# Developer-Zer0/GIF-synthesis-with-Discrete-Diffusion

Measured on AMD Instinct MI355X. Metric: 16-frame 128x128 videos/sec, 100-step D3PM sample, higher is better.
Workload: dtype f32; 1 GPU; C3: D3PM 100-step p_sample, guidance 2, 16x16x16 token grid, K=4096, 19 layers, bs 16/GPU + VQ-VAE decode to 3x16x128x128; global_batch=16, parallelism=replicas x1 (batch-sharded, no collective), hipgraph=True, sampler_lanes=2, weights=reference init N(0, 0.02)

## Files before the change

### gif-synthesis-with-discrete-diffusion_amd/_lib.py

```python
import ctypes as C
import os

import torch

_HERE = os.path.dirname(os.path.abspath(__file__))
LIB_PATH = os.environ.get("GSDD_LIB_PATH") or os.path.join(_HERE, "libgsdd.so")
_lib = None

EXPORTS = [
    "gsdd_last_error", "gsdd_version", "gsdd_abi_sizeof", "gsdd_gemm", "gsdd_row_stats", "gsdd_ncdhw_to_rows", "gsdd_preprocess_clip",
    "gsdd_axial_attention", "gsdd_pool3d", "gsdd_nearest_code", "gsdd_nearest_code_workspace_bytes", "gsdd_bn_train_workspace_bytes", "gsdd_bn_train",
    "gsdd_codebook_ema", "gsdd_code_perplexity", "gsdd_mse", "gsdd_conv_wgrad", "gsdd_bn_relu_bwd_workspace_bytes", "gsdd_bn_relu_bwd",
    "gsdd_relu_mask", "gsdd_lincomb", "gsdd_axial_attention_bwd", "gsdd_d3pm_embed", "gsdd_adaln_table", "gsdd_small_linear",
    "gsdd_d3pm_attention", "gsdd_d3pm_attention_workspace_bytes", "gsdd_d3pm_layer", "gsdd_d3pm_layer_pack", "gsdd_d3pm_layer_pack_h2", "gsdd_rows_linear_pack_many", "gsdd_rows_linear", "gsdd_d3pm_logits", "gsdd_d3pm_cross_attention", "gsdd_d3pm_step", "gsdd_d3pm_q_sample", "gsdd_d3pm_train_loss", "gsdd_d3pm_train_loss_bwd", "gsdd_d3pm_train_loss_grad", "gsdd_gelu2", "gsdd_ln_fwd", "gsdd_ln_bwd", "gsdd_wgrad",
    "gsdd_batch_rowsum", "gsdd_colsum", "gsdd_d3pm_attention_train", "gsdd_d3pm_attention_bwd", "gsdd_d3pm_attention_bwd_workspace_bytes", "gsdd_d3pm_embed_bwd", "gsdd_small_linear_bwd",
    "gsdd_adaln_bwd", "gsdd_adam", "gsdd_adam_multi", "gsdd_adam_multi_dev", "gsdd_advance", "gsdd_advance_floor",
    "gsdd_d3pm_purity_step", "gsdd_d3pm_purity_select", "gsdd_advance_plan",
    "gsdd_philox_uniform", "gsdd_graph_begin", "gsdd_graph_end", "gsdd_graph_launch", "gsdd_graph_destroy",
    "gsdd_event_create", "gsdd_event_record", "gsdd_event_elapsed_ms", "gsdd_event_destroy",
]

_p = C.c_void_p
_i = C.c_int
_i64 = C.c_int64
# ... 32 lines not shown
    ]


class PuritySelectDesc(C.Structure):
    _fields_ = [
        ("tok_in", _p), ("tok_out", _p), ("cand", _p), ("score", _p), ("smax", _p),
        ("B", _i), ("L", _i), ("K", _i), ("prior_rule", _i), ("n_dev", _p), ("seed", C.c_uint64), ("stream_dev", _p),
        ("stream_add", _i64), ("row0", _i64), ("key_dbg", _p),
    ]


class TrainDesc(C.Structure):
    _fields_ = [
        ("logits", _p), ("x0", _p), ("xt", _p), ("t_dev", _p), ("pt", _p),
        ("B", _i), ("L", _i), ("K", _i), ("T", _i), ("sched", _p * 8), ("mask_weight", C.c_float * 2),
        ("aux_weight", C.c_float), ("adaptive_aux", _i),
        ("kl", _p), ("nll", _p), ("aux", _p), ("x0_recon", _p), ("xt1_recon", _p),
        ("Lt_history", _p), ("Lt_count", _p), ("loss", _p), ("per_sample", _p), ("probs", _p),
    ]


class LayerDesc(C.Structure):
    _fields_ = [
        ("y", _p), ("x", _p), ("M", _i64), ("L", _i), ("n_embd", _i), ("hidden", _i), ("cvec", _p),
        ("wproj", _p), ("bproj", _p), ("ln2_g", _p), ("ln2_b", _p), ("w1", _p), ("b1", _p), ("w2", _p), ("b2", _p),
        ("ada", _p), ("t2", _p), ("wqkv", _p), ("bqkv", _p), ("qkv", _p), ("w2_x3", _p), ("wqkv_x3", _p), ("kv_img_bytes", _i64), ("kv_img", _p),
        ("layer_h2", _p), ("wqkv_h2", _p), ("variant", _i), ("range_flag", _p),
    ]


GEMM_EXACT_F32 = 1
AXIAL_AUTO, AXIAL_VALU = 0, 1
ATTN_AUTO, ATTN_P22, ATTN_P11, ATTN_A8, ATTN_A12, ATTN_F32PV, ATTN_KC256 = range(7)
LAYER_AUTO, LAYER_X3P, LAYER_H2 = 0, 2, 3
ATTN_BWD_AUTO, ATTN_BWD_VALU, ATTN_BWD_SPLIT, ATTN_BWD_FQC64, ATTN_BWD_FQC128, ATTN_BWD_NW8, ATTN_BWD_DBG1, ATTN_BWD_DBG2 = range(8)


class GsddError(RuntimeError):
    pass


def lib():
    global _lib
    if _lib is None:
        if not os.path.exists(LIB_PATH):
            raise GsddError(f"{LIB_PATH} is missing: the HIP extension must be built (./build.sh); "
                            "there is no CPU fallback for this path")
        L = C.CDLL(LIB_PATH)
        L.gsdd_last_error.restype = C.c_char_p
        if not hasattr(L, "gsdd_abi_sizeof"):
            raise GsddError(f"{LIB_PATH} predates this binding (no gsdd_abi_sizeof): rebuild it with ./build.sh")
        L.gsdd_abi_sizeof.argtypes, L.gsdd_abi_sizeof.restype = [_i], _i64
        for which, (name, cls) in enumerate((("gsdd_gemm_desc", GemmDesc), ("gsdd_layer_desc", LayerDesc), ("gsdd_step_desc", StepDesc),
                                             ("gsdd_train_desc", TrainDesc), ("gsdd_purity_desc", PurityDesc),
                                             ("gsdd_purity_select_desc", PuritySelectDesc))):
            if L.gsdd_abi_sizeof(which) != C.sizeof(cls):
                raise GsddError(f"{LIB_PATH} was built from another revision of include/gsdd.h: sizeof({name}) is {L.gsdd_abi_sizeof(which)} "
                                f"there and {C.sizeof(cls)} in this binding -- rebuild it with ./build.sh")
        L.gsdd_gemm.argtypes = [C.POINTER(GemmDesc), _p]
        L.gsdd_row_stats.argtypes = [_p, _i64, _i, C.c_float, _p, _p]
        L.gsdd_ncdhw_to_rows.argtypes = [_p, _i, _i, _i, _i, _i, _i, _i, _p, _p]
        L.gsdd_preprocess_clip.argtypes = [_p] + [_i] * 10 + [_p, _p]
        L.gsdd_axial_attention.argtypes = [_p, _i, _i, _i, _i, _i, _i, _p, _i, _p]
        L.gsdd_pool3d.argtypes = [_p, _i, _i, _i, _i, _i, _i, C.POINTER(_i), C.POINTER(_i), C.POINTER(_i), _i, _i, _i, _i, _p, _i, _p]
        L.gsdd_nearest_code.argtypes = [_p, _i64, _i, _p, _i, _p, _p, _p, _i64, _p]
        L.gsdd_nearest_code_workspace_bytes.argtypes = [_i]
# ... 85 lines not shown
```

### gif-synthesis-with-discrete-diffusion_amd/csrc/common.hpp

```cpp
#pragma once
#include <hip/hip_runtime.h>
#include <stdint.h>
#include <stdio.h>
#include <string.h>
#include <atomic>
#include <string>

#include "../../include/gsdd.h"

namespace gsdd {

void set_error(const std::string& s);

#define GSDD_CHECK_ARG(cond, msg)                                                      \
    do {                                                                               \
        if (!(cond)) {                                                                 \
            ::gsdd::set_error(std::string(__func__) + ": " + (msg) + " [" #cond "]"); \
            return GSDD_E_ARG;                                                         \
        }                                                                              \
    } while (0)

#define GSDD_CHECK_HIP(expr)                                                                   \
    do {                                                                                       \
        hipError_t e_ = (expr);                                                                \
// ... 101 lines not shown
        const float r1 = (vs[d] - (float)a) * 2048.f;
        const _Float16 b2 = (_Float16)r1;
        const float r2 = (r1 - (float)b2) * 2048.f;
        col[d] = a; col[4 + d] = b2; col[8 + d] = (_Float16)r2;
    }
    col[12] = (_Float16)1.f;
    col[13] = col[14] = col[15] = (_Float16)0.f;
    const int64_t pair = row >> 5;
    const int kk = (int)(row & 31), th = kk >> 4, kt = kk & 15, g = kt >> 2, r = kt & 3;
    _Float16* dst = reinterpret_cast<_Float16*>(vp + (pair * 4 + g) * 16) + 4 * th + r;
#pragma unroll
    for (int j = 0; j < 16; ++j) dst[j * 8] = col[j];
}

__host__ __device__ __forceinline__ float4* kv_image_ksum(void* workspace, int64_t rows) {
    return reinterpret_cast<float4*>(reinterpret_cast<char*>(workspace) + rows * 64);
}
__host__ __device__ __forceinline__ float* kv_image_knorm(void* workspace, int64_t rows) {
    return reinterpret_cast<float*>(reinterpret_cast<char*>(workspace) + rows * 64 + ((rows + 31) / 32) * 16);
}
template <int CTRL>
__device__ __forceinline__ float dpp_max(float v) {
    return fmaxf(v, __int_as_float(__builtin_amdgcn_update_dpp(0, __float_as_int(v), CTRL, 0xf, 0xf, true)));
}
template <int CTRL>
__device__ __forceinline__ float dpp_min(float v) {
    return fminf(v, __int_as_float(__builtin_amdgcn_update_dpp(__float_as_int(v), __float_as_int(v), CTRL, 0xf, 0xf, false)));
}
__device__ __forceinline__ float row16_max(float v) {
    v = dpp_max<0xB1>(v);
    v = dpp_max<0x4E>(v);
    v = dpp_max<0x141>(v);
    return dpp_max<0x140>(v);
}
__device__ __forceinline__ float row16_min(float v) {
    v = dpp_min<0xB1>(v);
    v = dpp_min<0x4E>(v);
    v = dpp_min<0x141>(v);
    return dpp_min<0x140>(v);
}
template <int CTRL>
__device__ __forceinline__ float dpp_add(float v) {
    return v + __int_as_float(__builtin_amdgcn_update_dpp(0, __float_as_int(v), CTRL, 0xf, 0xf, true));
}
__device__ __forceinline__ float dpp_prev_row_lane15(float v) {
    return __int_as_float(__builtin_amdgcn_update_dpp(0, __float_as_int(v), 0x142, 0xa, 0xf, false));
}
__device__ __forceinline__ float half32_sum(float v) {
    v = dpp_add<0xB1>(v);
    v = dpp_add<0x4E>(v);
    v = dpp_add<0x141>(v);
    v = dpp_add<0x140>(v);
    return v + dpp_prev_row_lane15(v);
}
__device__ __forceinline__ float half32_norm_bound(float n2) {
    float v = row16_max(n2);
    v = fmaxf(v, dpp_prev_row_lane15(v));
    return sqrtf(v) * 1.000001f + 1e-30f;
}
__device__ __forceinline__ void kv_image_store_knorm(const float4 (&o)[8], int h, int li, int64_t grp, int64_t M, float* knorm,
                                                     float4* ksum) {
#pragma unroll
    for (int q = 0; q < 8; ++q) {
        const float n2 = (o[q].x * o[q].x + o[q].y * o[q].y) + (o[q].z * o[q].z + o[q].w * o[q].w);
        const float nb = half32_norm_bound(n2);
        const float4 sk = make_float4(half32_sum(o[q].x), half32_sum(o[q].y), half32_sum(o[q].z), half32_sum(o[q].w));
// ... 16 lines not shown
```

### gif-synthesis-with-discrete-diffusion_amd/csrc/d3pm_attention.hip

```cpp
#include <stdlib.h>

#include <type_traits>

#include "common.hpp"

namespace gsdd {

typedef float f32x4 __attribute__((ext_vector_type(4)));
typedef __bf16 bf16x8 __attribute__((ext_vector_type(8)));

constexpr int KC = 256;
constexpr float RESCALE_THR = 40.f;

struct AttnSmem {
    uint4 k[2][KC][2];
    float v[2][KC / 4][4][4];
    uint4 ones[16];
};

__device__ __forceinline__ bf16x8 as_frag(uint4 u) {
    union { uint4 u; bf16x8 v; } c;
    c.u = u;
    return c.v;
}
// ... 313 lines not shown
            float p[8];
#pragma unroll
            for (int r = 0; r < 4; ++r) { p[r] = __builtin_amdgcn_exp2f(s0[r]); p[4 + r] = __builtin_amdgcn_exp2f(s1[r]); }
            uint4 hi, lo;
            if (MODE == 1) {
                split_p8(p, hi, lo);
                acc[j] = __builtin_amdgcn_mfma_f32_16x16x32_f16(as_h8(hi), vb, acc[j], 0, 0, 0);
                acc[j] = __builtin_amdgcn_mfma_f32_16x16x32_f16(as_h8(lo), vb, acc[j], 0, 0, 0);
            } else {
                round_p8(p, hi);
                acc[j] = __builtin_amdgcn_mfma_f32_16x16x32_f16(as_h8(hi), vb, acc[j], 0, 0, 0);
                if (MODE == 2) {
                    if (!MASK || !((skipmask[j] >> u) & 1u)) {
                        if (!MEASURE || __any(any_gt_h8(hi, thr2[j]))) {
                            resid_p8(p, hi, lo);
                            acc[j] = __builtin_amdgcn_mfma_f32_16x16x32_f16(as_h8(lo), vb, acc[j], 0, 0, 0);
                        } else {
                            ++skipped;
                        }
                    }
                }
            }
        }
    }
    return skipped;
}


template <int KC4, int PM = 1>
__global__ __launch_bounds__(256) void d3pm_attention_v4_kernel(const float* __restrict__ q, const uint4* __restrict__ kp,
                                                                const uint4* __restrict__ vp, const float* __restrict__ knorm,
                                                                const float4* __restrict__ ksum, int B, int L, int H,
                                                                float* __restrict__ out,
                                                                float* __restrict__ lse, unsigned long long* __restrict__ redo) {
    __shared__ AttnSmem4<KC4> sm;
    const int tid = threadIdx.x, lane = tid & 63, wave = tid >> 6;
    const int nqb = (L + 255) / 256;
    const unsigned nwg = gridDim.x;
    unsigned wg = blockIdx.x;
    {
        const unsigned q8 = nwg / 8, r8 = nwg % 8, xcd = wg % 8, idx = wg / 8;
        wg = (xcd < r8 ? xcd * (q8 + 1) : r8 * (q8 + 1) + (xcd - r8) * q8) + idx;
    }
    const int qblk = wg % nqb;
    const int h = (wg / nqb) % H, b = wg / (nqb * H);
    const int64_t M = (int64_t)B * L;
    const int64_t base = ((int64_t)h * M + (int64_t)b * L) * 4;
    const float* qh = q + base;
    const uint4* kph = kp + ((int64_t)h * M + (int64_t)b * L) * 2;
    const uint4* vph = vp + (((int64_t)h * M + (int64_t)b * L) >> 5) * 64;
    const float* knh = knorm + (((int64_t)h * M + (int64_t)b * L) >> 5);
    const float4* ksh = ksum + (((int64_t)h * M + (int64_t)b * L) >> 5);
    const int li = lane & 15, lg = lane >> 4;
    const int q0 = qblk * 256 + wave * 64;

    float knm = 0.f;
    float4 ks = make_float4(0.f, 0.f, 0.f, 0.f);
    if (PM >= 2) {
        for (int i = lane; i < (L >> 5); i += 64) {
            knm = fmaxf(knm, knh[i]);
            const float4 t = ksh[i];
            ks.x += t.x; ks.y += t.y; ks.z += t.z; ks.w += t.w;
        }
    }

    if (tid < 16) sm.ones[tid] = (tid == 0 || tid == 1) ? make_uint4(0x3F803F80u, 0x00003F80u, 0u, 0u) : make_uint4(0u, 0u, 0u, 0u);

    const float qscale = 0.5f * 1.4426950408889634f;
    uint4 qfrag[4];
    float rqn[4];
    float4 qsv[4];
#pragma unroll
    for (int j = 0; j < 4; ++j) {
        int qi = q0 + 16 * j + li;
        qi = qi < L ? qi : L - 1;
        const float4 qv = *reinterpret_cast<const float4*>(qh + (int64_t)qi * 4);
        const float qs[4] = {qv.x * qscale, qv.y * qscale, qv.z * qscale, qv.w * qscale};
        uint32_t q1[4], q2[4], q3[4];
#pragma unroll
        for (int d = 0; d < 4; ++d) split3(qs[d], q1[d], q2[d], q3[d]);
        const uint4 f0 = pack8(q1, q1), f1 = pack8(q2, q2), f2 = pack8(q1, q3);
        qfrag[j] = lg == 0 ? f0 : (lg == 1 ? f1 : (lg == 2 ? f2 : make_uint4(0u, 0u, 0u, 0u)));
        rqn[j] = 1.0f / (sqrtf((qs[0] * qs[0] + qs[1] * qs[1]) + (qs[2] * qs[2] + qs[3] * qs[3])) * 1.0001f + 1e-30f);
        qsv[j] = make_float4(qs[0], qs[1], qs[2], qs[3]);
    }

    const int nchunks = (L + KC4 - 1) / KC4;
    uint4 rk0, rk1, rk2, rv0, rv1, rv2;
    float rkn = 0.f, kn_cur = 0.f;
    auto load_chunk = [&](int c) {
        const int last = 2 * min(KC4, L - c * KC4) - 1;
        const uint4* ksrc = kph + (int64_t)c * KC4 * 2;
        const uint4* vsrc = vph + (int64_t)c * (KC4 / 32) * 64;
        rk0 = ksrc[min(tid, last)]; rk1 = ksrc[min(tid + 256, last)]; rk2 = ksrc[min(tid + 512, last)];
        rv0 = vsrc[min(tid, last)]; rv1 = vsrc[min(tid + 256, last)]; rv2 = vsrc[min(tid + 512, last)];
        if (PM >= 2) rkn = knh[min(c * (KC4 / 32) + min(lane, KC4 / 32 - 1), (L >> 5) - 1)];
    };
    auto store_chunk = [&](int buf, int) {
        uint4* kd = &sm.k[buf][0][0];
        uint4* vd = &sm.v[buf][0][0][0];
        kd[tid] = rk0; kd[tid + 256] = rk1; kd[tid + 512] = rk2;
        vd[tid] = rv0; vd[tid + 256] = rv1; vd[tid + 512] = rv2;
        kn_cur = rkn;
    };

    f32x4 acc[4], sav[4];
    float mq[4];
#pragma unroll
    for (int j = 0; j < 4; ++j) {
        mq[j] = 0.f;
        acc[j][0] = 0.f; acc[j][1] = 0.f; acc[j][2] = 0.f; acc[j][3] = 0.f;
    }
    const f32x4 zero = {0.f, 0.f, 0.f, 0.f};

    load_chunk(0);
    store_chunk(0, 0);
    __syncthreads();
    const int slot = ((lg >> 1) ^ (li >> 3)) & 1;
    const uint4* kbase0 = (lg == 3) ? &sm.ones[(li >= 4 && li < 12) ? 0 : 1] : &sm.k[0][li][slot];
    const int kstep = (lg == 3) ? 0 : 32;
    const int kbuf = (lg == 3) ? 0 : KC4 * 2;
    {
        const int nt0 = min(4, L >> 4);
#pragma unroll
        for (int j = 0; j < 4; ++j) {
            float m0 = -INFINITY;
            for (int t = 0; t < nt0; ++t) {
                const f32x4 s = __builtin_amdgcn_mfma_f32_16x16x32_bf16(as_frag(kbase0[t * kstep]), as_frag(qfrag[j]), zero, 0, 0, 0);
                m0 = fmaxf(m0, fmaxf(fmaxf(s[0], s[1]), fmaxf(s[2], s[3])));
            }
            m0 = fmaxf(m0, __shfl_xor(m0, 16));
            m0 = fmaxf(m0, __shfl_xor(m0, 32));
            mq[j] = ceilf(m0) - 3.f;
            if (lg == 3) qfrag[j] = negm_frag(mq[j]);
        }
    }

    bool prescan = false;
    bool adapt = PM >= 2;
    int probe = 1, backoff = 4;
    float jb[4] = {-INFINITY, -INFINITY, -INFINITY, -INFINITY};
    float kbj[4] = {0.f, 0.f, 0.f, 0.f};
    int kb_next = 1, kb_gap = 1;
    if (PM >= 2) {
        knm = wave_max(knm) * 1.0001f;
        const float budget = log2f((float)L) - (float)PM - 0.02f;
        ks.x = wave_sum(ks.x); ks.y = wave_sum(ks.y); ks.z = wave_sum(ks.z); ks.w = wave_sum(ks.w);
        const float invL = 1.0f / (float)L;
#pragma unroll
        for (int j = 0; j < 4; ++j) {
            const float dx = qsv[j].x * ks.x, dy = qsv[j].y * ks.y, dz = qsv[j].z * ks.z, dw = qsv[j].w * ks.w;
            const float mean = ((dx + dy) + (dz + dw)) * invL, mag = ((fabsf(dx) + fabsf(dy)) + (fabsf(dz) + fabsf(dw))) * invL;
            jb[j] = log2f((float)L) + mean - 1e-5f * mag - 0.02f;
            kbj[j] = row16_min(fmaxf(fmaxf(budget * rqn[j] - knm, (jb[j] - (float)PM) * rqn[j]), 0.f));
        }
    }
    for (int c = 0; c < nchunks; ++c) {
        const int buf = c & 1;
        if (c + 1 < nchunks) load_chunk(c + 1);
        const int npairs = min(KC4, L - c * KC4) >> 5;
        const uint4* kb = kbase0 + buf * kbuf;
#pragma unroll
        for (int j = 0; j < 4; ++j) sav[j] = acc[j];
        bool moved = false;
        for (int attempt = prescan ? -1 : 0; attempt < 16; ++attempt) {
          if (attempt >= 0) {
            uint32_t thr2[4] = {0u, 0u, 0u, 0u};
            uint32_t skipmask[4] = {0u, 0u, 0u, 0u};
            const uint32_t allmask = (1u << npairs) - 1u;
            if (PM >= 2) {
#pragma unroll
                for (int j = 0; j < 4; ++j) skipmask[j] = (uint32_t)__ballot(kn_cur < kbj[j]);
                const bool stale_clears = (skipmask[0] & skipmask[1] & skipmask[2] & skipmask[3] & allmask) == allmask;
                const bool refresh = !stale_clears && c >= kb_next;
                if (refresh) { kb_next = c + kb_gap; kb_gap *= 2; }
                if (refresh || (adapt && !stale_clears)) {
#pragma unroll
                    for (int j = 0; j < 4; ++j) {
                        const int src = ((li >> 2) << 4) + 12;
                        const float r0 = __shfl(sav[j][0], src), r1 = __shfl(sav[j][1], src), r2 = __shfl(sav[j][2], src),
                                    r3 = __shfl(sav[j][3], src);
                        const int rr = li & 3;
                        const float rs = rr == 0 ? r0 : (rr == 1 ? r1 : (rr == 2 ? r2 : r3));
                        if (refresh) {
                            float kbq = (__builtin_amdgcn_logf(rs) - (float)PM + mq[j] - 0.02f) * rqn[j];
                            kbq = fmaxf(kbq, 0.f);
                            kbj[j] = fmaxf(kbj[j], row16_min(kbq));

                            skipmask[j] = (uint32_t)__ballot(kn_cur < kbj[j]);
                        }
                        if (adapt && !stale_clears) {
                            const float rlb = fmaxf(rs, __builtin_amdgcn_exp2f(jb[j] - mq[j]));
// ... 2 lines not shown
                            thr2[j] = hb | (hb << 16);
                        }
                    }
                }
            }
            const uint32_t clr_all = skipmask[0] & skipmask[1] & skipmask[2] & skipmask[3] & allmask;
            int ncleared = 0;
#pragma unroll
            for (int j = 0; j < 4; ++j) ncleared += __builtin_popcount(skipmask[j] & allmask);
            int skipped = 0;
            const bool cleared = PM >= 2 && clr_all == allmask;
            if (PM == 0 || cleared) attn_tiles<KC4, 0>(sm, buf, npairs, kb, kstep, lg, li, qfrag, acc, thr2, skipmask);
            else if (PM == 1 || (!adapt && 2 * ncleared < 4 * npairs))
                attn_tiles<KC4, 1>(sm, buf, npairs, kb, kstep, lg, li, qfrag, acc, thr2, skipmask);
            else if (!adapt) skipped = ncleared + attn_tiles<KC4, 2, true, false>(sm, buf, npairs, kb, kstep, lg, li, qfrag, acc, thr2, skipmask);
            else if (ncleared == 0) skipped = attn_tiles<KC4, 2, false, true>(sm, buf, npairs, kb, kstep, lg, li, qfrag, acc, thr2, skipmask);
            else skipped = ncleared + attn_tiles<KC4, 2, true, true>(sm, buf, npairs, kb, kstep, lg, li, qfrag, acc, thr2, skipmask);
            float chk = 0.f;
#pragma unroll
            for (int j = 0; j < 4; ++j) chk += (acc[j][0] + acc[j][1]) + (acc[j][2] + acc[j][3]);
            const bool bad = !(fabsf(chk) < 3.0e38f);
            if (!__any(bad)) {
                if (PM >= 2 && !cleared) {
                    if (adapt) {
                        if (10 * skipped < 7 * 4 * npairs) { adapt = false; probe = backoff; backoff *= 2; }
                    } else if (--probe <= 0) {
                        adapt = true;
                    }
                }
                break;
            }
            moved = true;
            if (lane == 0 && redo != nullptr) atomicAdd(redo, 1ull);
          }
            const float trigger = attempt < 0 ? 12.f : 15.f;
            float cmax[4] = {-INFINITY, -INFINITY, -INFINITY, -INFINITY};
            for (int t = 0; t < 2 * npairs; ++t) {
                const bf16x8 kf = as_frag(kb[t * kstep]);
#pragma unroll
                for (int j = 0; j < 4; ++j) {
                    const f32x4 sx = __builtin_amdgcn_mfma_f32_16x16x32_bf16(kf, as_frag(qfrag[j]), zero, 0, 0, 0);
                    cmax[j] = fmaxf(cmax[j], fmaxf(fmaxf(sx[0], sx[1]), fmaxf(sx[2], sx[3])));
                }
            }
#pragma unroll
            for (int j = 0; j < 4; ++j) {
                float cm = fmaxf(cmax[j], __shfl_xor(cmax[j], 16));
                cm = fmaxf(cm, __shfl_xor(cm, 32));
                const float delta = cm >= trigger ? ceilf(cm) - 3.f : 0.f;
                if (attempt < 0 && __any(delta != 0.f)) moved = true;
                mq[j] += delta;
                if (lg == 3) qfrag[j] = negm_frag(mq[j]);
#pragma unroll
                for (int r = 0; r < 4; ++r) {
                    const float dr = __shfl(delta, (lane & 48) + 4 * lg + r);
                    acc[j][r] = sav[j][r] * __builtin_amdgcn_exp2f(-dr);
                }
                sav[j] = acc[j];
            }
        }
        prescan = moved;
        if (c + 1 < nchunks) store_chunk(buf ^ 1, c + 1);
        __syncthreads();
    }

#pragma unroll
    for (int j = 0; j < 4; ++j) {
#pragma unroll
        for (int r = 0; r < 4; ++r) {
            const float a = acc[j][r];
            const int rowbase = lane & 48;
            const float a1 = __shfl(a, rowbase + (li & 3) + 4);
            const float a2 = __shfl(a, rowbase + (li & 3) + 8);
            const float l = __shfl(a, rowbase + 12);
            const float mrow = __shfl(mq[j], rowbase + 4 * lg + r);
            const int qi = q0 + 16 * j + 4 * lg + r;
            if (li < 4 && qi < L) {
                const float o = (a + a1 * 0.00048828125f + a2 * 2.384185791015625e-07f) / l;
                out[((int64_t)b * L + qi) * (H * 4) + h * 4 + li] = o;
                if (lse != nullptr && li == 0) lse[(int64_t)h * M + (int64_t)b * L + qi] = mrow + log2f(l);
            }
        }
    }
}

__global__ void d3pm_cross_attention_kernel(const float* q, const float* kc, const float* vc, int B, int L, int Te, int H,
                                            float* out) {
    const int64_t M = (int64_t)B * L;
    const int64_t i = (int64_t)blockIdx.x * blockDim.x + threadIdx.x;
    if (i >= M * H) return;
    const int h = (int)(i / M);
    const int64_t m = i % M;
    const int b = (int)(m / L);
    const float4 qv = *reinterpret_cast<const float4*>(q + ((int64_t)h * M + m) * 4);
    float mx = -INFINITY;
    for (int e = 0; e < Te; ++e) {
        const float4 kv = *reinterpret_cast<const float4*>(kc + ((int64_t)b * Te + e) * (H * 4) + h * 4);
        const float s = (qv.x * kv.x + qv.y * kv.y + qv.z * kv.z + qv.w * kv.w) * 0.5f;
        mx = fmaxf(mx, s);
    }
    float l = 0.f, a0 = 0.f, a1 = 0.f, a2 = 0.f, a3 = 0.f;
    for (int e = 0; e < Te; ++e) {
        const float4 kv = *reinterpret_cast<const float4*>(kc + ((int64_t)b * Te + e) * (H * 4) + h * 4);
        const float4 vv = *reinterpret_cast<const float4*>(vc + ((int64_t)b * Te + e) * (H * 4) + h * 4);
        const float s = (qv.x * kv.x + qv.y * kv.y + qv.z * kv.z + qv.w * kv.w) * 0.5f;
        const float p = expf(s - mx);
        l += p;
        a0 += p * vv.x; a1 += p * vv.y; a2 += p * vv.z; a3 += p * vv.w;
    }
    const float inv = 1.0f / l;
    *reinterpret_cast<float4*>(out + m * (H * 4) + h * 4) = make_float4(a0 * inv, a1 * inv, a2 * inv, a3 * inv);
}

}

using namespace gsdd;

static int attn_p_mode(int mode, int L) {
    switch (mode) {
        case GSDD_ATTN_P22: return 1;
        case GSDD_ATTN_P11: return 0;
        case GSDD_ATTN_A8: return 8;
        case GSDD_ATTN_A12: return 12;
        default: return L >= 2048 ? 8 : 1;
    }
}

extern "C" int64_t gsdd_d3pm_attention_workspace_bytes(int B, int L, int H) {
    const int64_t rows = (int64_t)B * L * H;
    return rows * 64 + ((rows + 31) / 32) * 20;
}

int gsdd_attention_valu(const float* q, const float* k, const float* v, int B, int L, int H, float* out, float* lse,
                        void* stream);

extern "C" int gsdd_d3pm_attention(const float* q, const float* k, const float* v, int B, int L, int H, float* out,
                                   void* workspace, int64_t workspace_bytes, uint64_t* redo_events, int mode, void* stream) {
    GSDD_CHECK_ARG(q && out && ((k == nullptr) == (v == nullptr)), "null pointer");
    GSDD_CHECK_ARG(mode >= GSDD_ATTN_AUTO && mode <= GSDD_ATTN_KC256, "mode: one of GSDD_ATTN_*");
    GSDD_CHECK_ARG(B > 0 && H > 0 && L > 0, "bad sizes");
    GSDD_CHECK_ARG((int64_t)B * H * ((L + 255) / 256) < (1ll << 31), "grid too large");
    const bool premade = k == nullptr;
    const bool force_v3 = mode == GSDD_ATTN_F32PV;
    GSDD_CHECK_ARG(!premade || (L % 32 == 0 && workspace != nullptr && !force_v3), "k = v = NULL needs the matrix-pipe kernel's images in the workspace");
    if (L % 16 != 0) return gsdd_attention_valu(q, k, v, B, L, H, out, nullptr, stream);
    const dim3 grid((unsigned)(B * H * ((L + 255) / 256)));
    hipStream_t st = (hipStream_t)stream;
    if (L % 32 == 0 && !force_v3 && workspace != nullptr) {
        GSDD_CHECK_ARG(workspace_bytes >= gsdd_d3pm_attention_workspace_bytes(B, L, H), "workspace too small");
        const int64_t rows = (int64_t)B * L * H;
        uint4* kp = reinterpret_cast<uint4*>(workspace);
        uint4* vp = kp + rows * 2;
        float* kn = kv_image_knorm(workspace, rows);
        float4* ksm = kv_image_ksum(workspace, rows);
        unsigned long long* redo = reinterpret_cast<unsigned long long*>(redo_events);
        if (!premade) {
            hipLaunchKernelGGL(d3pm_attn_prep_kernel, dim3((unsigned)((rows + 255) / 256)), dim3(256), 0, st, k, v, rows, kp, vp, kn, ksm);
            GSDD_CHECK_LAUNCH();
        }
        const bool kc256 = mode == GSDD_ATTN_KC256;
        const int pmode = attn_p_mode(mode, L);
        float* nolse = nullptr;
        if (kc256) hipLaunchKernelGGL(d3pm_attention_v4_kernel<256>, grid, dim3(256), 0, st, q, kp, vp, kn, ksm, B, L, H, out, nolse, redo);
        else if (pmode == 0) hipLaunchKernelGGL((d3pm_attention_v4_kernel<384, 0>), grid, dim3(256), 0, st, q, kp, vp, kn, ksm, B, L, H, out, nolse, redo);
        else if (pmode == 8) hipLaunchKernelGGL((d3pm_attention_v4_kernel<384, 8>), grid, dim3(256), 0, st, q, kp, vp, kn, ksm, B, L, H, out, nolse, redo);
        else if (pmode == 12) hipLaunchKernelGGL((d3pm_attention_v4_kernel<384, 12>), grid, dim3(256), 0, st, q, kp, vp, kn, ksm, B, L, H, out, nolse, redo);
        else hipLaunchKernelGGL(d3pm_attention_v4_kernel<384>, grid, dim3(256), 0, st, q, kp, vp, kn, ksm, B, L, H, out, nolse, redo);
    } else {
        hipLaunchKernelGGL(d3pm_attention_kernel, grid, dim3(256), 0, st, q, k, v, B, L, H, out);
    }
    GSDD_CHECK_LAUNCH();
    return GSDD_OK;
}

int gsdd_attention_v4_with_lse(const float* q, const float* k, const float* v, int B, int L, int H, float* out, float* lse,
                               void* workspace, int64_t workspace_bytes, int mode, void* stream, int* done) {
    *done = 0;
    GSDD_CHECK_ARG(mode == GSDD_ATTN_AUTO || mode == GSDD_ATTN_P22 || mode == GSDD_ATTN_A8,
                   "training forward: mode is GSDD_ATTN_AUTO, GSDD_ATTN_P22 or GSDD_ATTN_A8");
    if (L % 32 != 0 || workspace == nullptr) return GSDD_OK;
    GSDD_CHECK_ARG(workspace_bytes >= gsdd_d3pm_attention_workspace_bytes(B, L, H), "workspace too small");
    GSDD_CHECK_ARG((int64_t)B * H * ((L + 255) / 256) < (1ll << 31), "grid too large");
    hipStream_t st = (hipStream_t)stream;
    const int64_t rows = (int64_t)B * L * H;
    uint4* kp = reinterpret_cast<uint4*>(workspace);
    uint4* vp = kp + rows * 2;
    float* kn = kv_image_knorm(workspace, rows);
    float4* ksm = kv_image_ksum(workspace, rows);
    unsigned long long* noredo = nullptr;
    hipLaunchKernelGGL(d3pm_attn_prep_kernel, dim3((unsigned)((rows + 255) / 256)), dim3(256), 0, st, k, v, rows, kp, vp, kn, ksm);
    GSDD_CHECK_LAUNCH();
    if (mode == GSDD_ATTN_A8 || (mode == GSDD_ATTN_AUTO && L >= 2048))
        hipLaunchKernelGGL((d3pm_attention_v4_kernel<384, 8>), dim3((unsigned)(B * H * ((L + 255) / 256))), dim3(256), 0, st, q, kp, vp, kn, ksm,
                           B, L, H, out, lse, noredo);
    else
        hipLaunchKernelGGL(d3pm_attention_v4_kernel<384>, dim3((unsigned)(B * H * ((L + 255) / 256))), dim3(256), 0, st, q, kp, vp, kn, ksm,
                           B, L, H, out, lse, noredo);
    GSDD_CHECK_LAUNCH();
    *done = 1;
    return GSDD_OK;
}

extern "C" int gsdd_d3pm_cross_attention(const float* q, const float* kc, const float* vc, int B, int L, int Te, int H,
                                         float* out, void* stream) {
    GSDD_CHECK_ARG(q && kc && vc && out, "null pointer");
    GSDD_CHECK_ARG(B > 0 && L > 0 && Te > 0 && H > 0, "bad sizes");
    const int64_t n = (int64_t)B * L * H;
    hipLaunchKernelGGL(d3pm_cross_attention_kernel, dim3((unsigned)((n + 255) / 256)), dim3(256), 0, (hipStream_t)stream,
                       q, kc, vc, B, L, Te, H, out);
    GSDD_CHECK_LAUNCH();
    return GSDD_OK;
}
```

### gif-synthesis-with-discrete-diffusion_amd/ops.py

```python
import ctypes as C
import os

import torch

from . import _lib as abi
from ._lib import GemmDesc, GsddError, LayerDesc, PurityDesc, PuritySelectDesc, StepDesc, TrainDesc, check, lib, ptr, stream_ptr

ACT_NONE, ACT_RELU, ACT_GELU2 = 0, 1, 2


_ATTN_MODES = {"auto": abi.ATTN_AUTO, "22": abi.ATTN_P22, "11": abi.ATTN_P11, "a8": abi.ATTN_A8, "a12": abi.ATTN_A12,
               "f32pv": abi.ATTN_F32PV, "kc256": abi.ATTN_KC256}
_LAYER_VARIANTS = {"auto": abi.LAYER_AUTO, "h2": abi.LAYER_H2, "x3p": abi.LAYER_X3P}
_ATTN_BWD_VARIANTS = {"auto": abi.ATTN_BWD_AUTO, "valu": abi.ATTN_BWD_VALU, "split": abi.ATTN_BWD_SPLIT, "fqc64": abi.ATTN_BWD_FQC64,
                      "fqc128": abi.ATTN_BWD_FQC128, "nw8": abi.ATTN_BWD_NW8, "dbg1": abi.ATTN_BWD_DBG1, "dbg2": abi.ATTN_BWD_DBG2}


def _pick(table, value, what):
    if isinstance(value, int):
        return value
    try:
        return table[str(value).lower()]
    except KeyError:
        raise GsddError(f"{what}: {value!r} is not one of {sorted(table)}") from None


def attn_mode(mode=None):
    if mode is not None:
        return _pick(_ATTN_MODES, mode, "attention mode")
    if os.environ.get("GSDD_ATTN_V3"):
        return abi.ATTN_F32PV
    if os.environ.get("GSDD_ATTN_KC") == "256":
        return abi.ATTN_KC256
    return _pick(_ATTN_MODES, os.environ.get("GSDD_ATTN_P", "auto"), "GSDD_ATTN_P")


def attn_train_mode(mode=None):
    v = mode if mode is not None else os.environ.get("GSDD_ATTN_TRAIN_P", "auto")
    m = _pick(_ATTN_MODES, v, "GSDD_ATTN_TRAIN_P")
    if m not in (abi.ATTN_AUTO, abi.ATTN_P22, abi.ATTN_A8):
        raise GsddError(f"GSDD_ATTN_TRAIN_P: {v!r} is not one of '22', 'a8'")
    return m


def attn_bwd_variant(variant=None):
    return _pick(_ATTN_BWD_VARIANTS, variant if variant is not None else os.environ.get("GSDD_ATTN_BWD", "auto"), "GSDD_ATTN_BWD")


def layer_variant(variant=None):
    return _pick(_LAYER_VARIANTS, variant if variant is not None else os.environ.get("GSDD_LAYER", "auto"), "GSDD_LAYER")


def gemm_flags(exact_f32=None):
    if exact_f32 is None:
        exact_f32 = bool(os.environ.get("GSDD_GEMM_F32"))
    return abi.GEMM_EXACT_F32 if exact_f32 else 0


def axial_variant(valu=None):
    if valu is None:
        valu = bool(os.environ.get("GSDD_AXIAL_VALU"))
    return abi.AXIAL_VALU if valu else abi.AXIAL_AUTO


def taps_tensor(taps, device):
    return torch.tensor(taps, dtype=torch.int32, device=device).contiguous()


def gemm(inp, w, out, *, in_dims, out_grid, stride=(1, 1, 1), taps=None, ntaps=1, cin=None, in_pitch=None,
         gather=None, pro=None, ln=None, epi_scale=None, epi_shift=None, bvec=None, rows_per_batch=0, act=ACT_NONE,
         residual=None, out_dims=None, out_step=(1, 1, 1), out_off=(0, 0, 0), out_pitch=None, out_mode=0, cout=None,
         exact_f32=None, stream=None, _desc_only=False):
    d = GemmDesc()
    N, Di, Hi, Wi = in_dims
    d.in_ = ptr(inp)
# ... 118 lines not shown
    return out[0]


def d3pm_embed(tok, emb, pos, x, rep=1, stream=None):
    B, L = tok.shape
    check(lib().gsdd_d3pm_embed(ptr(tok), B, L, emb.shape[1], ptr(emb), emb.shape[0], ptr(pos), rep, ptr(x),
                                stream_ptr(stream)))
    return x


def adaln_table(emb_w, lin_w, lin_b, out=None, stream=None):
    T, D = emb_w.shape
    if out is None:
        out = torch.empty((T, 2 * D), dtype=torch.float32, device=emb_w.device)
    check(lib().gsdd_adaln_table(ptr(emb_w), T, D, ptr(lin_w), ptr(lin_b), ptr(out), stream_ptr(stream)))
    return out


def small_linear(x, w, b, out=None, stream=None):
    R, Cin = x.shape
    if out is None:
        out = torch.empty((R, w.shape[0]), dtype=torch.float32, device=x.device)
    check(lib().gsdd_small_linear(ptr(x), R, Cin, ptr(w), ptr(b), w.shape[0], ptr(out), stream_ptr(stream)))
    return out


def d3pm_attention_workspace(B, L, H, device):
    n = lib().gsdd_d3pm_attention_workspace_bytes(B, L, H)
    return torch.empty(((n + 3) // 4,), dtype=torch.float32, device=device)


def d3pm_attention(q, k, v, B, L, H, out, ws=None, redo=None, mode=None, stream=None):
    nbytes = 0 if ws is None else ws.numel() * 4
    check(lib().gsdd_d3pm_attention(ptr(q), ptr(k), ptr(v), B, L, H, ptr(out), ptr(ws), nbytes, ptr(redo), attn_mode(mode),
                                    stream_ptr(stream)))
    return out


def d3pm_layer(y, x, L, lay, cvec=None, nxt=None, t2=None, qkv=None, kv_img=None, range_flag=None, variant=None, stream=None):
    d = LayerDesc()
    d.y, d.x, d.M, d.L, d.n_embd, d.hidden = ptr(y), ptr(x), x.shape[0], L, x.shape[1], 256
    d.cvec = ptr(cvec)
    if lay is not None:
        d.hidden = lay["w1"].shape[0]
        d.wproj, d.bproj, d.ln2_g, d.ln2_b = ptr(lay["wproj"]), ptr(lay["bproj"]), ptr(lay["g2"]), ptr(lay["b2"])
        d.w1, d.b1, d.w2, d.b2 = ptr(lay["w1"]), ptr(lay["bb1"]), ptr(lay["w2"]), ptr(lay["bb2"])
        d.w2_x3 = ptr(lay.get("w2_x3"))
        d.layer_h2 = ptr(lay.get("lay_h2"))
    if nxt is not None:
        d.ada, d.t2, d.wqkv, d.bqkv, d.qkv = ptr(nxt["ada1"]), ptr(t2), ptr(nxt["wqkv"]), ptr(nxt["bqkv"]), ptr(qkv)
        d.wqkv_x3 = ptr(nxt.get("wqkv_x3"))
        d.wqkv_h2 = ptr(nxt.get("wqkv_h2"))
        d.kv_img = ptr(kv_img)
        d.kv_img_bytes = 0 if kv_img is None else kv_img.numel() * kv_img.element_size()
    d.range_flag = ptr(range_flag)
    d.variant = layer_variant(variant)
    check(lib().gsdd_d3pm_layer(C.byref(d), stream_ptr(stream)))


LAYER_X3_BYTES, WQKV_X3_BYTES = 40 * 3 * 1024, 24 * 3 * 1024


def d3pm_layer_pack(w2, wproj, wqkv, stream=None):
    lay_x3 = torch.empty((LAYER_X3_BYTES,), dtype=torch.uint8, device=w2.device)
    wqkv_x3 = torch.empty((WQKV_X3_BYTES,), dtype=torch.uint8, device=w2.device)
    check(lib().gsdd_d3pm_layer_pack(ptr(w2), ptr(wproj), ptr(wqkv), ptr(lay_x3), ptr(wqkv_x3), stream_ptr(stream)))
    return lay_x3, wqkv_x3
# ... 226 lines not shown
    stats = torch.empty((x.shape[0], 2), dtype=torch.float32, device=x.device)
    y = torch.empty_like(x)
    check(lib().gsdd_ln_fwd(ptr(x), x.shape[0], x.shape[1], eps, ptr(gamma), ptr(beta), ptr(sel), gstride, rows_per_batch,
                            ptr(stats), ptr(y), stream_ptr(stream)))
    return stats, y


def ln_bwd(dh, x, stats, gamma, *, sel=None, gstride=0, rows_per_batch=1, dx_in=None, dgamma=None, dbeta=None,
           gacc_stride=0, acc_by_batch=False, stream=None):
    dx = torch.empty_like(x)
    check(lib().gsdd_ln_bwd(ptr(dh), ptr(x), ptr(stats), ptr(gamma), ptr(sel), gstride, rows_per_batch, x.shape[0], x.shape[1],
                            ptr(dx_in), ptr(dx), ptr(dgamma), ptr(dbeta), gacc_stride, int(acc_by_batch), stream_ptr(stream)))
    return dx


def wgrad(dY, X, dW, db=None, stream=None):
    check(lib().gsdd_wgrad(ptr(dY), dY.shape[1], ptr(X), X.shape[1], dY.shape[0], dY.shape[1], X.shape[1], ptr(dW), ptr(db),
                           stream_ptr(stream)))


def colsum(Y, out, stream=None):
    check(lib().gsdd_colsum(ptr(Y), Y.shape[1], Y.shape[0], Y.shape[1], ptr(out), stream_ptr(stream)))


def batch_rowsum(Y, B, L, out=None, stream=None):
    if out is None:
        out = torch.empty((B, Y.shape[1]), dtype=torch.float32, device=Y.device)
    check(lib().gsdd_batch_rowsum(ptr(Y), B, L, Y.shape[1], ptr(out), stream_ptr(stream)))
    return out


def d3pm_attention_train(q, k, v, B, L, H, out, lse, ws=None, mode=None, stream=None):
    check(lib().gsdd_d3pm_attention_train(ptr(q), ptr(k), ptr(v), B, L, H, ptr(out), ptr(lse), ptr(ws),
                                          0 if ws is None else ws.numel() * ws.element_size(), attn_train_mode(mode), stream_ptr(stream)))


def d3pm_attention_bwd_workspace(B, L, H, device):
    n = lib().gsdd_d3pm_attention_bwd_workspace_bytes(B, L, H)
    return torch.empty((n // 4,), dtype=torch.float32, device=device)


def d3pm_attention_bwd(q, k, v, o, dO, lse, B, L, H, ws=None, variant=None, stream=None):
    dqkv = torch.empty((B * L, 3 * H * 4), dtype=torch.float32, device=q.device)
    scratch = torch.empty((H * B * L,), dtype=torch.float32, device=q.device)
    check(lib().gsdd_d3pm_attention_bwd(ptr(q), ptr(k), ptr(v), ptr(o), ptr(dO), ptr(lse), B, L, H, ptr(dqkv), ptr(scratch), ptr(ws),
                                        0 if ws is None else ws.numel() * ws.element_size(), attn_bwd_variant(variant), stream_ptr(stream)))
    return dqkv


def d3pm_embed_bwd(dx, tok, demb, dpos, stream=None):
    B, L = tok.shape
    check(lib().gsdd_d3pm_embed_bwd(ptr(dx), ptr(tok), B, L, dx.shape[1], demb.shape[0], ptr(demb), ptr(dpos), stream_ptr(stream)))


def small_linear_bwd(dy, x, w, dw, db=None, want_dx=True, stream=None):
    R, Cin = x.shape
    dx = torch.empty_like(x) if want_dx else None
    check(lib().gsdd_small_linear_bwd(ptr(dy), ptr(x), ptr(w), R, Cin, w.shape[0], ptr(dx), ptr(dw), ptr(db), stream_ptr(stream)))
    return dx


def adaln_bwd(dtab, t, emb, w, demb, dw, db, stream=None):
    check(lib().gsdd_adaln_bwd(ptr(dtab), ptr(t), dtab.shape[0], emb.shape[1], ptr(emb), ptr(w), ptr(demb), ptr(dw), ptr(db),
                               stream_ptr(stream)))


def adam(p, g, m, v, lr, beta1, beta2, eps, step, stream=None):
# ... 38 lines not shown
```

### include/gsdd.h

```cpp
#ifndef GSDD_H
#define GSDD_H
#include <stdint.h>

#ifdef __cplusplus
extern "C" {
#endif

#define GSDD_OK 0
#define GSDD_E_ARG (-1)
#define GSDD_E_HIP (-2)
#define GSDD_E_STATE (-3)

const char* gsdd_last_error(void);
int gsdd_version(void);
int64_t gsdd_abi_sizeof(int which);

typedef struct {
    const float* in;
    int N, Di, Hi, Wi, Cin, in_pitch;
    int Do, Ho, Wo;
    int sd, sh, sw;
    int ntaps;
    const int* taps;
    const int64_t* gather;
// ... 48 lines not shown

int gsdd_code_perplexity(const float* n_local, int K, int64_t M, float* out, void* stream);

int gsdd_mse(const float* a, const float* b, int64_t n, float scale, float* out, void* workspace, int64_t workspace_bytes,
             void* stream);

int gsdd_conv_wgrad(const gsdd_gemm_desc* d, const float* dY, int dy_pitch, float* dW, void* stream);
int64_t gsdd_bn_relu_bwd_workspace_bytes(int64_t M, int C);
int gsdd_bn_relu_bwd(const float* da, const float* x, int64_t M, int C, const float* mean_rstd, const float* gamma,
                     const float* beta, const float* dx_in, float* dx, float* dgamma, float* dbeta, void* workspace,
                     int64_t workspace_bytes, void* stream);
int gsdd_relu_mask(const float* dout, const float* out, float* dpre, int64_t n, void* stream);
int gsdd_lincomb(const float* a, const float* b, const float* c, float alpha, float* out, int64_t n, void* stream);
int gsdd_axial_attention_bwd(const float* qkv, const float* datt, int N, int T, int H, int W, int C, int n_head, float* dqkv,
                             int variant , void* stream);

int gsdd_d3pm_embed(const int64_t* tok, int B, int L, int D, const float* emb, int n_embed,
                    const float* pos, int rep, float* x, void* stream);

int gsdd_adaln_table(const float* emb, int T, int D, const float* lin_w, const float* lin_b,
                     float* out, void* stream);

int gsdd_small_linear(const float* x, int R, int Cin, const float* w, const float* b, int Cout,
                      float* y, void* stream);

int64_t gsdd_d3pm_attention_workspace_bytes(int B, int L, int H);
#define GSDD_ATTN_AUTO 0
#define GSDD_ATTN_P22 1
#define GSDD_ATTN_P11 2
#define GSDD_ATTN_A8 3
#define GSDD_ATTN_A12 4
#define GSDD_ATTN_F32PV 5
#define GSDD_ATTN_KC256 6
int gsdd_d3pm_attention(const float* q, const float* k, const float* v, int B, int L, int H,
                        float* out, void* workspace, int64_t workspace_bytes, uint64_t* redo_events, int mode, void* stream);

typedef struct {
    const float* y;
    float* x;
    int64_t M;
    int L;
    int n_embd, hidden;
    const float* cvec;
    const float* wproj; const float* bproj;
    const float* ln2_g; const float* ln2_b;
    const float* w1; const float* b1;
    const float* w2; const float* b2;
    const float* ada;
    const int64_t* t2;
    const float* wqkv; const float* bqkv;
    float* qkv;
    const void* w2_x3;
    const void* wqkv_x3;
    int64_t kv_img_bytes;
    void* kv_img;
    const void* layer_h2;
    const void* wqkv_h2;
    int variant;
    int* range_flag;
} gsdd_layer_desc;
#define GSDD_LAYER_AUTO 0
#define GSDD_LAYER_X3P 2
#define GSDD_LAYER_H2 3
int gsdd_d3pm_layer(const gsdd_layer_desc* d, void* stream);
#define GSDD_LAYER_X3_BYTES (40 * 3 * 1024)
#define GSDD_LAYER_WQKV_X3_BYTES (24 * 3 * 1024)
// ... 160 lines not shown
```

Before: 7.808 videos/s.

## Add lean attention fast path skipping adaptive rescale bookkeeping when bounds prove safe

Adds a block-wide 'quiet' check in the v4 attention kernel. If the precomputed key-norm and query-norm bounds guarantee no overflow or rescale, every chunk runs through a plain tile loop without the per-chunk key-norm loads and the adaptive probe/rescale logic. It also moves the key-norm and key-sum reductions into wave 0 and shares them through shared memory, drops index clamping on full chunks, caps the redo loop, and rewrites the epilogue to use DPP moves instead of shuffles. The fast path is on by default and can be disabled with an env flag. The risk is that a wrong bound check lets precision issues pass unnoticed.

```diff
diff --git a/gif-synthesis-with-discrete-diffusion_amd/_lib.py b/gif-synthesis-with-discrete-diffusion_amd/_lib.py
--- a/gif-synthesis-with-discrete-diffusion_amd/_lib.py
+++ b/gif-synthesis-with-discrete-diffusion_amd/_lib.py
@@ -88,6 +88,7 @@
 GEMM_EXACT_F32 = 1
 AXIAL_AUTO, AXIAL_VALU = 0, 1
 ATTN_AUTO, ATTN_P22, ATTN_P11, ATTN_A8, ATTN_A12, ATTN_F32PV, ATTN_KC256 = range(7)
+ATTN_NOLEAN = 256
 LAYER_AUTO, LAYER_X3P, LAYER_H2 = 0, 2, 3
 ATTN_BWD_AUTO, ATTN_BWD_VALU, ATTN_BWD_SPLIT, ATTN_BWD_FQC64, ATTN_BWD_FQC128, ATTN_BWD_NW8, ATTN_BWD_DBG1, ATTN_BWD_DBG2 = range(8)
 
diff --git a/gif-synthesis-with-discrete-diffusion_amd/csrc/common.hpp b/gif-synthesis-with-discrete-diffusion_amd/csrc/common.hpp
--- a/gif-synthesis-with-discrete-diffusion_amd/csrc/common.hpp
+++ b/gif-synthesis-with-discrete-diffusion_amd/csrc/common.hpp
@@ -157,6 +157,10 @@
     v = dpp_max<0x4E>(v);
     v = dpp_max<0x141>(v);
     return dpp_max<0x140>(v);
+}
+template <int CTRL>
+__device__ __forceinline__ float dpp_mov(float v) {
+    return __int_as_float(__builtin_amdgcn_update_dpp(0, __float_as_int(v), CTRL, 0xf, 0xf, true));
 }
 __device__ __forceinline__ float row16_min(float v) {
     v = dpp_min<0xB1>(v);
diff --git a/gif-synthesis-with-discrete-diffusion_amd/csrc/d3pm_attention.hip b/gif-synthesis-with-discrete-diffusion_amd/csrc/d3pm_attention.hip
--- a/gif-synthesis-with-discrete-diffusion_amd/csrc/d3pm_attention.hip
+++ b/gif-synthesis-with-discrete-diffusion_amd/csrc/d3pm_attention.hip
@@ -369,7 +369,7 @@
                                                                 const uint4* __restrict__ vp, const float* __restrict__ knorm,
                                                                 const float4* __restrict__ ksum, int B, int L, int H,
                                                                 float* __restrict__ out,
-                                                                float* __restrict__ lse, unsigned long long* __restrict__ redo) {
+                                                                float* __restrict__ lse, unsigned long long* __restrict__ redo, int lean) {
     __shared__ AttnSmem4<KC4> sm;
     const int tid = threadIdx.x, lane = tid & 63, wave = tid >> 6;
     const int nqb = (L + 255) / 256;
@@ -393,9 +393,12 @@
 
     float knm = 0.f;
     float4 ks = make_float4(0.f, 0.f, 0.f, 0.f);
-    if (PM >= 2) {
+    bool kn_odd = false;
+    if (PM >= 2 && wave == 0) {
         for (int i = lane; i < (L >> 5); i += 64) {
-            knm = fmaxf(knm, knh[i]);
+            const float n = knh[i];
+            knm = fmaxf(knm, n);
+            kn_odd = kn_odd || !(n < 3.0e38f);
             const float4 t = ksh[i];
             ks.x += t.x; ks.y += t.y; ks.z += t.z; ks.w += t.w;
         }
@@ -406,6 +409,7 @@
     const float qscale = 0.5f * 1.4426950408889634f;
     uint4 qfrag[4];
     float rqn[4];
+    float qn[4];
     float4 qsv[4];
 #pragma unroll
     for (int j = 0; j < 4; ++j) {
@@ -418,20 +422,29 @@
         for (int d = 0; d < 4; ++d) split3(qs[d], q1[d], q2[d], q3[d]);
         const uint4 f0 = pack8(q1, q1), f1 = pack8(q2, q2), f2 = pack8(q1, q3);
         qfrag[j] = lg == 0 ? f0 : (lg == 1 ? f1 : (lg == 2 ? f2 : make_uint4(0u, 0u, 0u, 0u)));
-        rqn[j] = 1.0f / (sqrtf((qs[0] * qs[0] + qs[1] * qs[1]) + (qs[2] * qs[2] + qs[3] * qs[3])) * 1.0001f + 1e-30f);
+        qn[j] = sqrtf((qs[0] * qs[0] + qs[1] * qs[1]) + (qs[2] * qs[2] + qs[3] * qs[3])) * 1.0001f + 1e-30f;
+        rqn[j] = 1.0f / qn[j];
         qsv[j] = make_float4(qs[0], qs[1], qs[2], qs[3]);
     }
 
     const int nchunks = (L + KC4 - 1) / KC4;
     uint4 rk0, rk1, rk2, rv0, rv1, rv2;
     float rkn = 0.f, kn_cur = 0.f;
-    auto load_chunk = [&](int c) {
-        const int last = 2 * min(KC4, L - c * KC4) - 1;
+    const unsigned so0 = (unsigned)tid, so1 = (unsigned)tid + 256u, so2 = (unsigned)tid + 512u;
+    auto load_chunk = [&](int c, bool norms) {
+        const int rem = L - c * KC4;
         const uint4* ksrc = kph + (int64_t)c * KC4 * 2;
         const uint4* vsrc = vph + (int64_t)c * (KC4 / 32) * 64;
-        rk0 = ksrc[min(tid, last)]; rk1 = ksrc[min(tid + 256, last)]; rk2 = ksrc[min(tid + 512, last)];
-        rv0 = vsrc[min(tid, last)]; rv1 = vsrc[min(tid + 256, last)]; rv2 = vsrc[min(tid + 512, last)];
-        if (PM >= 2) rkn = knh[min(c * (KC4 / 32) + min(lane, KC4 / 32 - 1), (L >> 5) - 1)];
+        if (2 * KC4 == 768 && rem >= KC4) {
+            rk0 = ksrc[so0]; rk1 = ksrc[so1]; rk2 = ksrc[so2];
+            rv0 = vsrc[so0]; rv1 = vsrc[so1]; rv2 = vsrc[so2];
+        } else {
+            const unsigned last = 2u * (unsigned)rem - 1u;
+            const unsigned c0 = min(so0, last), c1 = min(so1, last), c2 = min(so2, last);
+            rk0 = ksrc[c0]; rk1 = ksrc[c1]; rk2 = ksrc[c2];
+            rv0 = vsrc[c0]; rv1 = vsrc[c1]; rv2 = vsrc[c2];
+        }
+        if (PM >= 2 && norms) rkn = knh[min(c * (KC4 / 32) + min(lane, KC4 / 32 - 1), (L >> 5) - 1)];
     };
     auto store_chunk = [&](int buf, int) {
         uint4* kd = &sm.k[buf][0][0];
@@ -450,7 +463,16 @@
     }
     const f32x4 zero = {0.f, 0.f, 0.f, 0.f};
 
-    load_chunk(0);
+    load_chunk(0, true);
+    if (PM >= 2 && wave == 0) {
+        knm = wave_max(knm);
+        ks.x = wave_sum(ks.x); ks.y = wave_sum(ks.y); ks.z = wave_sum(ks.z); ks.w = wave_sum(ks.w);
+        const bool odd = __any(kn_odd);
+        if (lane == 0) {
+            sm.ones[2] = make_uint4(__float_as_uint(ks.x), __float_as_uint(ks.y), __float_as_uint(ks.z), __float_as_uint(ks.w));
+            sm.ones[3] = make_uint4(__float_as_uint(knm), odd ? 1u : 0u, 0u, 0u);
+        }
+    }
     store_chunk(0, 0);
     __syncthreads();
     const int slot = ((lg >> 1) ^ (li >> 3)) & 1;
@@ -474,27 +496,47 @@
     }
 
     bool prescan = false;
+    bool quiet = false;
     bool adapt = PM >= 2;
     int probe = 1, backoff = 4;
     float jb[4] = {-INFINITY, -INFINITY, -INFINITY, -INFINITY};
     float kbj[4] = {0.f, 0.f, 0.f, 0.f};
     int kb_next = 1, kb_gap = 1;
     if (PM >= 2) {
-        knm = wave_max(knm) * 1.0001f;
+        const uint4 shk = sm.ones[2], shn = sm.ones[3];
+        knm = __uint_as_float(shn.x) * 1.0001f;
+        ks = make_float4(__uint_as_float(shk.x), __uint_as_float(shk.y), __uint_as_float(shk.z), __uint_as_float(shk.w));
         const float budget = log2f((float)L) - (float)PM - 0.02f;
-        ks.x = wave_sum(ks.x); ks.y = wave_sum(ks.y); ks.z = wave_sum(ks.z); ks.w = wave_sum(ks.w);
         const float invL = 1.0f / (float)L;
 #pragma unroll
         for (int j = 0; j < 4; ++j) {
             const float dx = qsv[j].x * ks.x, dy = qsv[j].y * ks.y, dz = qsv[j].z * ks.z, dw = qsv[j].w * ks.w;
             const float mean = ((dx + dy) + (dz + dw)) * invL, mag = ((fabsf(dx) + fabsf(dy)) + (fabsf(dz) + fabsf(dw))) * invL;
             jb[j] = log2f((float)L) + mean - 1e-5f * mag - 0.02f;
-            kbj[j] = row16_min(fmaxf(fmaxf(budget * rqn[j] - knm, (jb[j] - (float)PM) * rqn[j]), 0.f));
-        }
-    }
+            const float kbq0 = fmaxf(fmaxf(budget * rqn[j] - knm, (jb[j] - (float)PM) * rqn[j]), 0.f);
+            kbj[j] = row16_min(qn[j] != qn[j] ? INFINITY : kbq0);
+        }
+        if (lean != 0) {
+            bool ok = shn.y == 0u;
+#pragma unroll
+            for (int j = 0; j < 4; ++j) ok = ok && (knm < kbj[j]) && (qn[j] * knm - mq[j] <= 15.f);
+            quiet = __all(ok);
+        }
+    }
+    if (PM >= 2 && quiet) {
+        const uint32_t none[4] = {0u, 0u, 0u, 0u};
+        for (int c = 0; c < nchunks; ++c) {
+            const int buf = c & 1;
+            if (c + 1 < nchunks) load_chunk(c + 1, false);
+            const int npairs = min(KC4, L - c * KC4) >> 5;
+            attn_tiles<KC4, 0>(sm, buf, npairs, kbase0 + buf * kbuf, kstep, lg, li, qfrag, acc, none, none);
+            if (c + 1 < nchunks) store_chunk(buf ^ 1, c + 1);
+            __syncthreads();
+        }
+    } else
     for (int c = 0; c < nchunks; ++c) {
         const int buf = c & 1;
-        if (c + 1 < nchunks) load_chunk(c + 1);
+        if (c + 1 < nchunks) load_chunk(c + 1, true);
         const int npairs = min(KC4, L - c * KC4) >> 5;
         const uint4* kb = kbase0 + buf * kbuf;
 #pragma unroll
@@ -563,6 +605,7 @@
             }
             moved = true;
             if (lane == 0 && redo != nullptr) atomicAdd(redo, 1ull);
+            if (attempt == 15) break;
           }
             const float trigger = attempt < 0 ? 12.f : 15.f;
             float cmax[4] = {-INFINITY, -INFINITY, -INFINITY, -INFINITY};
@@ -595,21 +638,37 @@
         __syncthreads();
     }
 
+    const unsigned orow = (unsigned)(H * 16);
+    const unsigned ovo = (unsigned)(4 * lg) * orow + (unsigned)(li * 4);
+    char* const ob = reinterpret_cast<char*>(out + ((int64_t)b * L + q0) * (H * 4) + h * 4);
 #pragma unroll
     for (int j = 0; j < 4; ++j) {
+        if (q0 + 16 * j >= L) break;
+        float a1[4], a2[4], l[4];
 #pragma unroll
         for (int r = 0; r < 4; ++r) {
-            const float a = acc[j][r];
-            const int rowbase = lane & 48;
-            const float a1 = __shfl(a, rowbase + (li & 3) + 4);
-            const float a2 = __shfl(a, rowbase + (li & 3) + 8);
-            const float l = __shfl(a, rowbase + 12);
-            const float mrow = __shfl(mq[j], rowbase + 4 * lg + r);
-            const int qi = q0 + 16 * j + 4 * lg + r;
-            if (li < 4 && qi < L) {
-                const float o = (a + a1 * 0.00048828125f + a2 * 2.384185791015625e-07f) / l;
-                out[((int64_t)b * L + qi) * (H * 4) + h * 4 + li] = o;
-                if (lse != nullptr && li == 0) lse[(int64_t)h * M + (int64_t)b * L + qi] = mrow + log2f(l);
+            a1[r] = dpp_mov<0x104>(acc[j][r]);
+            a2[r] = dpp_mov<0x108>(acc[j][r]);
+            l[r] = dpp_mov<0x10C>(dpp_mov<0x00>(acc[j][r]));
+        }
+        if (li < 4) {
+#pragma unroll
+            for (int r = 0; r < 4; ++r) {
+                const float o = (acc[j][r] + a1[r] * 0.00048828125f + a2[r] * 2.384185791015625e-07f) / l[r];
+                *reinterpret_cast<float*>(ob + (ovo + (unsigned)(16 * j + r) * orow)) = o;
+            }
+        }
+    }
+    if (lse != nullptr) {
+        char* const lb = reinterpret_cast<char*>(lse + (int64_t)h * M + (int64_t)b * L + q0);
+#pragma unroll
+        for (int j = 0; j < 4; ++j) {
+            if (q0 + 16 * j >= L) break;
+#pragma unroll
+            for (int r = 0; r < 4; ++r) {
+                const float l = dpp_mov<0x10C>(dpp_mov<0x00>(acc[j][r]));
+                const float mrow = __shfl(mq[j], (lane & 48) + 4 * lg + r);
+                if (li == 0) *reinterpret_cast<float*>(lb + (unsigned)(4 * (16 * j + r) + 16 * lg)) = mrow + log2f(l);
             }
         }
     }
@@ -668,6 +727,8 @@
 extern "C" int gsdd_d3pm_attention(const float* q, const float* k, const float* v, int B, int L, int H, float* out,
                                    void* workspace, int64_t workspace_bytes, uint64_t* redo_events, int mode, void* stream) {
     GSDD_CHECK_ARG(q && out && ((k == nullptr) == (v == nullptr)), "null pointer");
+    const int lean = (mode & GSDD_ATTN_NOLEAN) ? 0 : 1;
+    mode &= ~GSDD_ATTN_NOLEAN;
     GSDD_CHECK_ARG(mode >= GSDD_ATTN_AUTO && mode <= GSDD_ATTN_KC256, "mode: one of GSDD_ATTN_*");
     GSDD_CHECK_ARG(B > 0 && H > 0 && L > 0, "bad sizes");
     GSDD_CHECK_ARG((int64_t)B * H * ((L + 255) / 256) < (1ll << 31), "grid too large");
@@ -692,11 +753,11 @@
         const bool kc256 = mode == GSDD_ATTN_KC256;
         const int pmode = attn_p_mode(mode, L);
         float* nolse = nullptr;
-        if (kc256) hipLaunchKernelGGL(d3pm_attention_v4_kernel<256>, grid, dim3(256), 0, st, q, kp, vp, kn, ksm, B, L, H, out, nolse, redo);
-        else if (pmode == 0) hipLaunchKernelGGL((d3pm_attention_v4_kernel<384, 0>), grid, dim3(256), 0, st, q, kp, vp, kn, ksm, B, L, H, out, nolse, redo);
-        else if (pmode == 8) hipLaunchKernelGGL((d3pm_attention_v4_kernel<384, 8>), grid, dim3(256), 0, st, q, kp, vp, kn, ksm, B, L, H, out, nolse, redo);
-        else if (pmode == 12) hipLaunchKernelGGL((d3pm_attention_v4_kernel<384, 12>), grid, dim3(256), 0, st, q, kp, vp, kn, ksm, B, L, H, out, nolse, redo);
-        else hipLaunchKernelGGL(d3pm_attention_v4_kernel<384>, grid, dim3(256), 0, st, q, kp, vp, kn, ksm, B, L, H, out, nolse, redo);
+        if (kc256) hipLaunchKernelGGL(d3pm_attention_v4_kernel<256>, grid, dim3(256), 0, st, q, kp, vp, kn, ksm, B, L, H, out, nolse, redo, lean);
+        else if (pmode == 0) hipLaunchKernelGGL((d3pm_attention_v4_kernel<384, 0>), grid, dim3(256), 0, st, q, kp, vp, kn, ksm, B, L, H, out, nolse, redo, lean);
+        else if (pmode == 8) hipLaunchKernelGGL((d3pm_attention_v4_kernel<384, 8>), grid, dim3(256), 0, st, q, kp, vp, kn, ksm, B, L, H, out, nolse, redo, lean);
+        else if (pmode == 12) hipLaunchKernelGGL((d3pm_attention_v4_kernel<384, 12>), grid, dim3(256), 0, st, q, kp, vp, kn, ksm, B, L, H, out, nolse, redo, lean);
+        else hipLaunchKernelGGL(d3pm_attention_v4_kernel<384>, grid, dim3(256), 0, st, q, kp, vp, kn, ksm, B, L, H, out, nolse, redo, lean);
     } else {
         hipLaunchKernelGGL(d3pm_attention_kernel, grid, dim3(256), 0, st, q, k, v, B, L, H, out);
     }
@@ -707,6 +768,8 @@
 int gsdd_attention_v4_with_lse(const float* q, const float* k, const float* v, int B, int L, int H, float* out, float* lse,
                                void* workspace, int64_t workspace_bytes, int mode, void* stream, int* done) {
     *done = 0;
+    const int lean = (mode & GSDD_ATTN_NOLEAN) ? 0 : 1;
+    mode &= ~GSDD_ATTN_NOLEAN;
     GSDD_CHECK_ARG(mode == GSDD_ATTN_AUTO || mode == GSDD_ATTN_P22 || mode == GSDD_ATTN_A8,
                    "training forward: mode is GSDD_ATTN_AUTO, GSDD_ATTN_P22 or GSDD_ATTN_A8");
     if (L % 32 != 0 || workspace == nullptr) return GSDD_OK;
@@ -723,10 +786,10 @@
     GSDD_CHECK_LAUNCH();
     if (mode == GSDD_ATTN_A8 || (mode == GSDD_ATTN_AUTO && L >= 2048))
         hipLaunchKernelGGL((d3pm_attention_v4_kernel<384, 8>), dim3((unsigned)(B * H * ((L + 255) / 256))), dim3(256), 0, st, q, kp, vp, kn, ksm,
-                           B, L, H, out, lse, noredo);
+                           B, L, H, out, lse, noredo, lean);
     else
         hipLaunchKernelGGL(d3pm_attention_v4_kernel<384>, dim3((unsigned)(B * H * ((L + 255) / 256))), dim3(256), 0, st, q, kp, vp, kn, ksm,
-                           B, L, H, out, lse, noredo);
+                           B, L, H, out, lse, noredo, lean);
     GSDD_CHECK_LAUNCH();
     *done = 1;
     return GSDD_OK;
diff --git a/gif-synthesis-with-discrete-diffusion_amd/ops.py b/gif-synthesis-with-discrete-diffusion_amd/ops.py
--- a/gif-synthesis-with-discrete-diffusion_amd/ops.py
+++ b/gif-synthesis-with-discrete-diffusion_amd/ops.py
@@ -41,6 +41,13 @@
     if m not in (abi.ATTN_AUTO, abi.ATTN_P22, abi.ATTN_A8):
         raise GsddError(f"GSDD_ATTN_TRAIN_P: {v!r} is not one of '22', 'a8'")
     return m
+
+
+def attn_lean_flag():
+    v = os.environ.get("GSDD_ATTN_LEAN", "1")
+    if v not in ("0", "1"):
+        raise GsddError(f"GSDD_ATTN_LEAN: {v!r} is not one of '0', '1'")
+    return abi.ATTN_NOLEAN if v == "0" else 0
 
 
 def attn_bwd_variant(variant=None):
@@ -225,7 +232,7 @@
 
 def d3pm_attention(q, k, v, B, L, H, out, ws=None, redo=None, mode=None, stream=None):
     nbytes = 0 if ws is None else ws.numel() * 4
-    check(lib().gsdd_d3pm_attention(ptr(q), ptr(k), ptr(v), B, L, H, ptr(out), ptr(ws), nbytes, ptr(redo), attn_mode(mode),
+    check(lib().gsdd_d3pm_attention(ptr(q), ptr(k), ptr(v), B, L, H, ptr(out), ptr(ws), nbytes, ptr(redo), attn_mode(mode) | attn_lean_flag(),
                                     stream_ptr(stream)))
     return out
 
@@ -518,7 +525,7 @@
 
 def d3pm_attention_train(q, k, v, B, L, H, out, lse, ws=None, mode=None, stream=None):
     check(lib().gsdd_d3pm_attention_train(ptr(q), ptr(k), ptr(v), B, L, H, ptr(out), ptr(lse), ptr(ws),
-                                          0 if ws is None else ws.numel() * ws.element_size(), attn_train_mode(mode), stream_ptr(stream)))
+                                          0 if ws is None else ws.numel() * ws.element_size(), attn_train_mode(mode) | attn_lean_flag(), stream_ptr(stream)))
 
 
 def d3pm_attention_bwd_workspace(B, L, H, device):
diff --git a/include/gsdd.h b/include/gsdd.h
--- a/include/gsdd.h
+++ b/include/gsdd.h
@@ -104,6 +104,7 @@
 #define GSDD_ATTN_A12 4
 #define GSDD_ATTN_F32PV 5
 #define GSDD_ATTN_KC256 6
+#define GSDD_ATTN_NOLEAN 256
 int gsdd_d3pm_attention(const float* q, const float* k, const float* v, int B, int L, int H,
                         float* out, void* workspace, int64_t workspace_bytes, uint64_t* redo_events, int mode, void* stream);
 
```

Measured after the change: 8.188 videos/s (median of 6 runs). +4.9%, better.
